# horovod/horovod

Hardware: AMD Instinct MI355X
Metric: images/sec, ResNet-50 synthetic (total over all GPUs) (higher is better)
Workload: dtype bf16; 1 GPU; model=resnet50, global_batch=64, image_size=224, parallelism=dp1, compression=none, reduction=average, optimizer=sgd, fused_sgd=True, fused_bn=False, hipgraph=False

## Files before the change

### csrc/bindings.cc

```cpp
#include <torch/extension.h>

#include "core.h"
#include "timeline.h"
#include "gpu.h"

namespace {

using namespace hvd;

ReduceOp OpFromInt(int op) { return (ReduceOp)op; }

py::tuple WaitHandle(int handle) {
  std::vector<at::Tensor> outputs;
  at::Tensor extra;
  int32_t result_int = -1;
  Status s;
  {
    py::gil_scoped_release nogil;
    s = State().handles.Wait(handle, outputs, extra, &result_int);
  }
  if (!s.ok()) {
    if (s.type == StatusType::ABORTED)
      throw std::runtime_error("HorovodInternalError: " + s.reason);
    throw std::runtime_error(s.reason);
// ... 201 lines not shown
          return hvd::gpu::FusedLarsStep(params, grads, momenta, lr, momentum,
                                         weight_decay, trust_coefficient, eps,
                                         nesterov, trust_clip, adapt,
                                         opt_tensor(grad_coef),
                                         opt_list(model_params),
                                         opt_tensor(skip));
        },
        py::arg("params"), py::arg("grads"), py::arg("momenta"),
        py::arg("lr"), py::arg("momentum"), py::arg("weight_decay"),
        py::arg("trust_coefficient"), py::arg("eps"), py::arg("nesterov"),
        py::arg("trust_clip"), py::arg("adapt"),
        py::arg("grad_coef") = py::none(),
        py::arg("model_params") = py::none(), py::arg("skip") = py::none());

  m.def("fused_bn_relu_forward",
        [](at::Tensor x, py::object residual, at::Tensor gamma, at::Tensor beta,
           at::Tensor rm, at::Tensor rv, double momentum, double eps) {
          at::Tensor res;
          if (!residual.is_none()) res = residual.cast<at::Tensor>();
          return hvd::gpu::FusedBnReluForward(x, res, gamma, beta, rm, rv,
                                              momentum, eps);
        });
  m.def("fused_bn_relu_backward",
        [](at::Tensor x, at::Tensor y, at::Tensor dy, at::Tensor mean,
           at::Tensor invstd, at::Tensor gamma, bool need_res) {
          return hvd::gpu::FusedBnReluBackward(x, y, dy, mean, invstd, gamma,
                                               need_res);
        });
  m.def("fused_bn_pass",
        [](int which, at::Tensor x, py::object a, py::object b, py::object out,
           at::Tensor mean, at::Tensor invstd, at::Tensor gamma,
           at::Tensor beta) {
          auto opt = [](const py::object& o) {
            return o.is_none() ? at::Tensor() : o.cast<at::Tensor>();
          };
          hvd::gpu::FusedBnPass(which, x, opt(a), opt(b), opt(out), mean,
                                invstd, gamma, beta);
        });

  m.def("sync_bn_stats",
        [](at::Tensor x) { return hvd::gpu::SyncBnStats(x); });
  m.def("sync_bn_normalize",
        [](at::Tensor x, at::Tensor stats, py::object weight, py::object bias,
           py::object rm, py::object rv, double momentum, double eps) {
          auto opt = [](const py::object& o) {
            return o.is_none() ? at::Tensor() : o.cast<at::Tensor>();
          };
          return hvd::gpu::SyncBnNormalize(x, stats, opt(weight), opt(bias),
                                           opt(rm), opt(rv), momentum, eps);
        });
  m.def("sync_bn_backward_reduce",
// ... 41 lines not shown
```

### csrc/bn_common.h

```cpp
#pragma once

#include <hip/hip_runtime.h>
#include <hip/hip_fp16.h>
#include <hip/hip_bf16.h>

#include <algorithm>
#include <cstdint>

#include "kernels.h"

namespace hvd {
namespace gpu {
namespace {

template <typename T>
__device__ __forceinline__ float to_f(T v) { return (float)v; }
template <>
__device__ __forceinline__ float to_f<__hip_bfloat16>(__hip_bfloat16 v) {
  return __bfloat162float(v);
}
template <typename T>
__device__ __forceinline__ T from_f(float v) { return (T)v; }
template <>
__device__ __forceinline__ __hip_bfloat16 from_f<__hip_bfloat16>(float v) {
  return __float2bfloat16(v);
}

template <typename T>
union Vec8 {
  uint4 u[2];
  T e[8];
  __device__ Vec8() {}
};

template <typename T>
__device__ __forceinline__ void load8(Vec8<T>& v, const T* p, long long i) {
  if (sizeof(T) == 2) {
    v.u[0] = ((const uint4*)p)[i];
  } else {
    v.u[0] = ((const uint4*)p)[i * 2];
    v.u[1] = ((const uint4*)p)[i * 2 + 1];
  }
}

template <typename T>
__device__ __forceinline__ void store8(T* p, long long i, const Vec8<T>& v) {
  if (sizeof(T) == 2) {
    ((uint4*)p)[i] = v.u[0];
// ... 80 lines not shown
```

### csrc/bn_kernels.hip

```cpp
#include "bn_common.h"
#include "kernels.h"

namespace hvd {
namespace gpu {

namespace {

template <typename T>
__global__ __launch_bounds__(256) void bn_stats_k(const T* __restrict__ x,
                                                  long long total, int C,
                                                  float* __restrict__ banks) {
  extern __shared__ float lds[];
  for (int c = threadIdx.x; c < 2 * C; c += blockDim.x) lds[c] = 0.f;
  __syncthreads();
  const long long tid = (long long)blockIdx.x * blockDim.x + threadIdx.x;
  const long long nthreads = (long long)gridDim.x * blockDim.x;
  const long long nvec = total / 8;
  const int c0 = octet_channel(C);
  float rsum[8] = {0}, rsq[8] = {0};
  auto add = [&](const Vec8<T>& v) {
#pragma unroll
    for (int k = 0; k < 8; ++k) {
      float f = to_f<T>(v.e[k]);
      rsum[k] += f;
// ... 21 lines not shown
}

template <typename T, bool ADD>
__global__ __launch_bounds__(256) void bn_apply_relu_k(
    const T* __restrict__ x, const T* __restrict__ res, T* __restrict__ y,
    const float* __restrict__ mean, const float* __restrict__ invstd,
    const float* __restrict__ gamma, const float* __restrict__ beta,
    long long total, int C) {
  const long long tid = (long long)blockIdx.x * blockDim.x + threadIdx.x;
  const long long nthreads = (long long)gridDim.x * blockDim.x;
  const long long nvec = total / 8;
  const int c0 = octet_channel(C);
  float rm[8], ri[8], rg[8], rb[8];
  load_octet(rm, mean, c0, 0.f);
  load_octet(ri, invstd, c0, 0.f);
  load_octet(rg, gamma, c0, 1.f);
  load_octet(rb, beta, c0, 0.f);
  for (long long i = tid; i < nvec; i += nthreads) {
    Vec8<T> vx, vr, vy;
    load8(vx, x, i);
    if (ADD) load8(vr, res, i);
#pragma unroll
    for (int k = 0; k < 8; ++k) {
      float f = (to_f<T>(vx.e[k]) - rm[k]) * ri[k] * rg[k] + rb[k];
      if (ADD) f += to_f<T>(vr.e[k]);
      vy.e[k] = from_f<T>(f > 0.f ? f : 0.f);
    }
    store8(y, i, vy);
  }
}

template <typename T, bool WRITE_G>
__global__ __launch_bounds__(256) void bn_bwd_stats_k(
    const T* __restrict__ x, const T* __restrict__ y, const T* __restrict__ dy,
    T* __restrict__ g_out, const float* __restrict__ mean,
    const float* __restrict__ invstd, long long total, int C,
    float* __restrict__ banks) {
  extern __shared__ float lds[];
  for (int c = threadIdx.x; c < 2 * C; c += blockDim.x) lds[c] = 0.f;
  __syncthreads();
  const long long tid = (long long)blockIdx.x * blockDim.x + threadIdx.x;
  const long long nthreads = (long long)gridDim.x * blockDim.x;
  const long long nvec = total / 8;
  const int c0 = octet_channel(C);
  float rmean[8], racc_g[8] = {0}, racc_gx[8] = {0};
  load_octet(rmean, mean, c0, 0.f);
  for (long long i = tid; i < nvec; i += nthreads) {
    Vec8<T> vx, vy, vd, vg;
    load8(vx, x, i);
    load8(vy, y, i);
    load8(vd, dy, i);
#pragma unroll
    for (int k = 0; k < 8; ++k) {
      float gv = to_f<T>(vy.e[k]) > 0.f ? to_f<T>(vd.e[k]) : 0.f;
      racc_g[k] += gv;
      racc_gx[k] += gv * (to_f<T>(vx.e[k]) - rmean[k]);
      if (WRITE_G) vg.e[k] = from_f<T>(gv);
    }
    if (WRITE_G) store8(g_out, i, vg);
  }
  float rinv[8];
  load_octet(rinv, invstd, c0, 0.f);
#pragma unroll
  for (int k = 0; k < 8; ++k) racc_gx[k] *= rinv[k];
  octet_flush(racc_g, racc_gx, c0, C, lds, banks);
}

__global__ __launch_bounds__(256) void bn_bank_reduce_k(float* banks,
                                                        int C) {
  for (int c = blockIdx.x * blockDim.x + threadIdx.x; c < 2 * C;
       c += gridDim.x * blockDim.x) {
    float acc = 0.f;
    for (int b = 0; b < kBnBanks; ++b) acc += banks[(size_t)b * 2 * C + c];
    banks[c] = acc;
  }
}

template <typename T, bool FROM_G>
__global__ __launch_bounds__(256) void bn_bwd_apply_k(
    const T* __restrict__ x, const T* __restrict__ y, const T* __restrict__ dy,
    T* __restrict__ dx, const float* __restrict__ mean,
    const float* __restrict__ invstd, const float* __restrict__ gamma,
    const float* __restrict__ sum_g, const float* __restrict__ sum_gx,
    long long total, int C, float inv_count) {
  const long long tid = (long long)blockIdx.x * blockDim.x + threadIdx.x;
  const long long nthreads = (long long)gridDim.x * blockDim.x;
  const long long nvec = total / 8;
  const int c0 = octet_channel(C);
  float rmean[8], rinv[8], rgi[8], rsg[8], rsgx[8];
  load_octet(rmean, mean, c0, 0.f);
  load_octet(rinv, invstd, c0, 0.f);
  load_octet(rgi, gamma, c0, 1.f);
  load_octet(rsg, sum_g, c0, 0.f);
  load_octet(rsgx, sum_gx, c0, 0.f);
#pragma unroll
  for (int k = 0; k < 8; ++k) {
    rgi[k] = rgi[k] * rinv[k];
    rsg[k] = rsg[k] * inv_count;
    rsgx[k] = rsgx[k] * inv_count;
  }
  for (long long i = tid; i < nvec; i += nthreads) {
    Vec8<T> vx, vy, vd, vo;
    load8(vx, x, i);
    if (!FROM_G) load8(vy, y, i);
    load8(vd, dy, i);
#pragma unroll
    for (int k = 0; k < 8; ++k) {
      float gv = FROM_G ? to_f<T>(vd.e[k])
                        : (to_f<T>(vy.e[k]) > 0.f ? to_f<T>(vd.e[k]) : 0.f);
      float xh = (to_f<T>(vx.e[k]) - rmean[k]) * rinv[k];
      float v = rgi[k] * (gv - rsg[k] - xh * rsgx[k]);
      vo.e[k] = from_f<T>(v);
    }
    store8(dx, i, vo);
  }
}

__global__ __launch_bounds__(256) void bn_finalize_k(
    const float* __restrict__ banks, float* __restrict__ mean,
    float* __restrict__ invstd, float* __restrict__ running_mean,
    float* __restrict__ running_var, long long count, float momentum,
    float eps, int C) {
  const int c = blockIdx.x * blockDim.x + threadIdx.x;
  if (c >= C) return;
  const float inv_n = 1.0f / (float)count;
  const float ub = count > 1 ? (float)count / (float)(count - 1) : 1.0f;
  float s = 0.f, q = 0.f;
#pragma unroll 16
  for (int b = 0; b < kBnBanks; ++b) {
    s += banks[(size_t)b * 2 * C + c];
    q += banks[(size_t)b * 2 * C + C + c];
  }
  float m = s * inv_n;
  float v = q * inv_n - m * m;
  mean[c] = m;
  invstd[c] = rsqrtf(v + eps);
  if (running_mean) {
    running_mean[c] = (1.f - momentum) * running_mean[c] + momentum * m;
    running_var[c] = (1.f - momentum) * running_var[c] + momentum * v * ub;
  }
}

template <size_t N>
bool aligned16(const void* const (&ptrs)[N]) {
  return aligned_to(ptrs, (int)N, 16);
}

}

#define DISPATCH_T(DT, FN)                                        \
  switch (DT) {                                                   \
    case DT_F32: { using scalar_t = float; FN; break; }           \
    case DT_F16: { using scalar_t = __half; FN; break; }          \
    case DT_BF16: { using scalar_t = __hip_bfloat16; FN; break; } \
    default: return hipErrorInvalidValue;                         \
  }

hipError_t BnFinalizeLaunch(const float* banks, float* mean, float* invstd,
                            float* running_mean, float* running_var,
                            long long count, float momentum, float eps,
                            int C, hipStream_t stream) {
  bn_finalize_k<<<(C + 255) / 256, 256, 0, stream>>>(
      banks, mean, invstd, running_mean, running_var, count, momentum, eps, C);
  return hipGetLastError();
}

hipError_t BnBankReduceLaunch(float* banks, int C, hipStream_t stream) {
  int blocks = (2 * C + 255) / 256;
  bn_bank_reduce_k<<<blocks, 256, 0, stream>>>(banks, C);
  return hipGetLastError();
}

hipError_t BnStatsLaunch(const void* x, long long total, int C, int dt,
                         float* banks, hipStream_t stream) {
  const void* const ptrs[] = {x};
  if (!aligned16(ptrs)) return hipErrorInvalidValue;
  int blocks = vec8_reduce_grid(total, C);
  size_t lds = 2 * (size_t)C * sizeof(float);
  DISPATCH_T(dt, (bn_stats_k<scalar_t><<<blocks, 256, lds, stream>>>(
                     (const scalar_t*)x, total, C, banks)));
  return hipGetLastError();
}

hipError_t BnApplyReluLaunch(const void* x, const void* res, void* y,
                             const float* mean, const float* invstd,
                             const float* gamma, const float* beta,
                             long long total, int C, int dt,
                             hipStream_t stream) {
  const void* const ptrs[] = {x, res, y, mean, invstd, gamma, beta};
  if (!aligned16(ptrs)) return hipErrorInvalidValue;
  int blocks = grid_for(total, C);
  if (res) {
    DISPATCH_T(dt, (bn_apply_relu_k<scalar_t, true><<<blocks, 256, 0, stream>>>(
                       (const scalar_t*)x, (const scalar_t*)res, (scalar_t*)y,
                       mean, invstd, gamma, beta, total, C)));
  } else {
    DISPATCH_T(dt,
               (bn_apply_relu_k<scalar_t, false><<<blocks, 256, 0, stream>>>(
                   (const scalar_t*)x, nullptr, (scalar_t*)y, mean, invstd,
                   gamma, beta, total, C)));
  }
  return hipGetLastError();
}

hipError_t BnBwdStatsLaunch(const void* x, const void* y, const void* dy,
                            void* g_out, const float* mean,
                            const float* invstd, long long total, int C,
                            int dt, float* banks, hipStream_t stream) {
  const void* const ptrs[] = {x, y, dy, g_out, mean, invstd};
  if (!aligned16(ptrs)) return hipErrorInvalidValue;
  int blocks = vec8_reduce_grid(total, C);
  size_t lds = 2 * (size_t)C * sizeof(float);
  if (g_out) {
    DISPATCH_T(dt,
               (bn_bwd_stats_k<scalar_t, true><<<blocks, 256, lds, stream>>>(
                   (const scalar_t*)x, (const scalar_t*)y, (const scalar_t*)dy,
                   (scalar_t*)g_out, mean, invstd, total, C, banks)));
  } else {
    DISPATCH_T(dt,
               (bn_bwd_stats_k<scalar_t, false><<<blocks, 256, lds, stream>>>(
                   (const scalar_t*)x, (const scalar_t*)y, (const scalar_t*)dy,
                   nullptr, mean, invstd, total, C, banks)));
  }
  return hipGetLastError();
}

hipError_t BnBwdApplyLaunch(const void* x, const void* y, const void* dy,
                            void* dx, const float* mean, const float* invstd,
                            const float* gamma, const float* sum_g,
                            const float* sum_gx, long long total, int C,
                            int dt, float inv_count, hipStream_t stream) {
  const void* const ptrs[] = {x,      y,     dy,    dx,    mean,
                              invstd, gamma, sum_g, sum_gx};
  if (!aligned16(ptrs)) return hipErrorInvalidValue;
  int blocks = grid_for(total, C);
  if (y) {
    DISPATCH_T(dt, (bn_bwd_apply_k<scalar_t, false><<<blocks, 256, 0, stream>>>(
                       (const scalar_t*)x, (const scalar_t*)y,
                       (const scalar_t*)dy, (scalar_t*)dx, mean, invstd, gamma,
                       sum_g, sum_gx, total, C, inv_count)));
  } else {
    DISPATCH_T(dt, (bn_bwd_apply_k<scalar_t, true><<<blocks, 256, 0, stream>>>(
                       (const scalar_t*)x, nullptr, (const scalar_t*)dy,
                       (scalar_t*)dx, mean, invstd, gamma, sum_g, sum_gx,
                       total, C, inv_count)));
  }
  return hipGetLastError();
}

#undef DISPATCH_T

}
}
```

### csrc/gpu.cc

```cpp
#include "gpu.h"

#include <hip/hip_runtime_api.h>
#include <rccl/rccl.h>
#include <roctracer/roctx.h>

#include <c10/hip/HIPCachingAllocator.h>
#include <c10/hip/HIPGuard.h>
#include <c10/hip/HIPStream.h>

#include <algorithm>
#include <condition_variable>
#include <cstring>
#include <deque>
#include <mutex>
#include <stdexcept>
#include <thread>
#include <unordered_map>

#include "core.h"
#include "hip_check.h"
#include "kernels.h"
#include "logging.h"
#include "timeline.h"

// ... 1323 lines not shown
    HIP_CHECK(AdasumDotsLaunch(args, dt, dots + start * 3, stream));
  }
  for (size_t start = 0; start < a.size(); start += kCopyBatchCapacity) {
    AdasumBatchArgs args;
    args.count = (int)std::min<size_t>(kCopyBatchCapacity, a.size() - start);
    for (int k = 0; k < args.count; ++k) {
      args.a[k] = a[start + k].data_ptr();
      args.b[k] = b[start + k].data_ptr();
      args.numel[k] = (unsigned long long)a[start + k].numel();
    }
    HIP_CHECK(AdasumScaledAddLaunch(args, dt, dots + start * 3, stream));
  }
}

namespace {

at::Tensor BnParamF32(const at::Tensor& t) {
  if (t.scalar_type() == at::kFloat && t.is_contiguous() &&
      (uintptr_t)t.data_ptr() % 16 == 0)
    return t;
  return t.to(at::kFloat).clone(at::MemoryFormat::Contiguous);
}

}

std::vector<at::Tensor> FusedBnReluForward(at::Tensor x, at::Tensor residual,
                                           at::Tensor gamma, at::Tensor beta,
                                           at::Tensor running_mean,
                                           at::Tensor running_var,
                                           double momentum, double eps) {
  TORCH_CHECK(x.dim() == 4, "fused BN expects NCHW logical 4-D input");
  TORCH_CHECK(x.is_contiguous(at::MemoryFormat::ChannelsLast),
              "fused BN requires channels_last layout");
  int64_t C = x.size(1);
  TORCH_CHECK(C % 8 == 0 && C <= 4096, "fused BN requires C % 8 == 0, C <= 4096");
  TORCH_CHECK(gamma.numel() == C && beta.numel() == C,
              "fused BN: weight and bias must have C elements");
  TORCH_CHECK(!residual.defined() ||
                  (residual.sizes() == x.sizes() &&
                   residual.scalar_type() == x.scalar_type() &&
                   residual.is_contiguous(at::MemoryFormat::ChannelsLast)),
              "fused BN: residual must match x in shape, dtype and layout");
  int device = (int)x.get_device();
  c10::hip::HIPGuard guard(device);
  hipStream_t stream = c10::hip::getCurrentHIPStream(device).stream();
  int64_t total = x.numel();
  int64_t count = total / C;
  int dt = (int)DataTypeFromTorch(x.scalar_type());

  auto fopts = at::TensorOptions().dtype(at::kFloat).device(x.device());
  const int64_t bank_elems = (int64_t)kBnBanks * 2 * C;
  at::Tensor ws = at::empty({bank_elems + 2 * C}, fopts);
  float* wsp = ws.data_ptr<float>();
  float* mean_p = wsp + bank_elems;
  float* invstd_p = mean_p + C;
  HIP_CHECK(hipMemsetAsync(wsp, 0, (size_t)bank_elems * sizeof(float),
                           stream));
  HIP_CHECK(BnStatsLaunch(x.data_ptr(), total, (int)C, dt, wsp, stream));
  TORCH_CHECK(!running_mean.defined() ||
                  (running_var.defined() && running_mean.numel() == C &&
                   running_var.numel() == C),
              "fused BN: running stats must have C elements");
  bool stats_f32 = running_mean.defined() &&
                   running_mean.scalar_type() == at::kFloat &&
                   running_mean.is_contiguous() &&
                   running_var.scalar_type() == at::kFloat &&
                   running_var.is_contiguous();
  HIP_CHECK(BnFinalizeLaunch(
      wsp, mean_p, invstd_p,
      stats_f32 ? running_mean.data_ptr<float>() : nullptr,
      stats_f32 ? running_var.data_ptr<float>() : nullptr, count,
      (float)momentum, (float)eps, (int)C, stream));
  at::Tensor mean = ws.narrow(0, bank_elems, C);
  at::Tensor invstd = ws.narrow(0, bank_elems + C, C);
  if (!stats_f32 && running_mean.defined()) {
    at::Tensor var = at::pow(invstd, -2) - eps;
    running_mean.mul_(1 - momentum).add_(mean.to(running_mean.scalar_type()),
                                         momentum);
    double ub = count > 1 ? (double)count / (count - 1) : 1.0;
    running_var.mul_(1 - momentum)
        .add_((var * ub).to(running_var.scalar_type()), momentum);
  }
  at::Tensor gamma_f = BnParamF32(gamma);
  at::Tensor beta_f = BnParamF32(beta);
  at::Tensor y = at::empty_like(x);
  HIP_CHECK(BnApplyReluLaunch(
      x.data_ptr(), residual.defined() ? residual.data_ptr() : nullptr,
      y.data_ptr(), mean_p, invstd_p, gamma_f.data_ptr<float>(),
      beta_f.data_ptr<float>(), total, (int)C, dt, stream));
  return {y, mean, invstd};
}

std::vector<at::Tensor> FusedBnReluBackward(at::Tensor x, at::Tensor y,
                                            at::Tensor dy, at::Tensor mean,
                                            at::Tensor invstd, at::Tensor gamma,
                                            bool need_residual_grad) {
  int device = (int)x.get_device();
  c10::hip::HIPGuard guard(device);
  hipStream_t stream = c10::hip::getCurrentHIPStream(device).stream();
  int64_t C = x.size(1);
  int64_t total = x.numel();
  int64_t count = total / C;
  int dt = (int)DataTypeFromTorch(x.scalar_type());
  if (!dy.is_contiguous(at::MemoryFormat::ChannelsLast))
    dy = dy.contiguous(at::MemoryFormat::ChannelsLast);
  TORCH_CHECK(x.dim() == 4 && C % 8 == 0 && C <= 4096 &&
                  x.is_contiguous(at::MemoryFormat::ChannelsLast) &&
                  y.is_contiguous(at::MemoryFormat::ChannelsLast),
              "fused BN backward: x and y must be channels_last with "
              "C % 8 == 0, C <= 4096");
  TORCH_CHECK(y.sizes() == x.sizes() && dy.sizes() == x.sizes() &&
                  y.scalar_type() == x.scalar_type() &&
                  dy.scalar_type() == x.scalar_type() &&
                  mean.numel() == C && invstd.numel() == C &&
                  gamma.numel() == C,
              "fused BN backward: mismatched shapes or dtypes");

  auto fopts = at::TensorOptions().dtype(at::kFloat).device(x.device());
  at::Tensor sums = at::empty({(int64_t)kBnBanks * 2 * C}, fopts);
  float* bankp = sums.data_ptr<float>();
  HIP_CHECK(hipMemsetAsync(bankp, 0,
                           (size_t)kBnBanks * 2 * C * sizeof(float), stream));
  at::Tensor dres;
  if (need_residual_grad) dres = at::empty_like(x);
  at::Tensor mean_f = BnParamF32(mean), invstd_f = BnParamF32(invstd);
  HIP_CHECK(BnBwdStatsLaunch(x.data_ptr(), y.data_ptr(), dy.data_ptr(),
                             need_residual_grad ? dres.data_ptr() : nullptr,
                             mean_f.data_ptr<float>(),
                             invstd_f.data_ptr<float>(), total, (int)C, dt,
                             bankp, stream));
  HIP_CHECK(BnBankReduceLaunch(bankp, (int)C, stream));
  at::Tensor gamma_f = BnParamF32(gamma);
  at::Tensor dx = at::empty_like(x);
  HIP_CHECK(BnBwdApplyLaunch(
      x.data_ptr(), need_residual_grad ? nullptr : y.data_ptr(),
      need_residual_grad ? dres.data_ptr() : dy.data_ptr(), dx.data_ptr(),
      mean_f.data_ptr<float>(), invstd_f.data_ptr<float>(),
      gamma_f.data_ptr<float>(), bankp, bankp + C, total, (int)C, dt,
      (float)(1.0 / count), stream));
  at::Tensor sum_g = sums.narrow(0, 0, C), sum_gx = sums.narrow(0, C, C);
  at::Tensor dbeta = gamma.scalar_type() == at::kFloat
                         ? sum_g
                         : sum_g.to(gamma.scalar_type());
  at::Tensor dgamma = gamma.scalar_type() == at::kFloat
                          ? sum_gx
                          : sum_gx.to(gamma.scalar_type());
  std::vector<at::Tensor> out{dx, dgamma, dbeta};
  if (need_residual_grad) out.push_back(dres);
  return out;
}

void FusedBnPass(int which, at::Tensor x, at::Tensor a, at::Tensor b,
                 at::Tensor out, at::Tensor mean, at::Tensor invstd,
                 at::Tensor gamma, at::Tensor beta) {
  TORCH_CHECK(x.dim() == 4 && x.is_contiguous(at::MemoryFormat::ChannelsLast),
              "fused BN requires channels_last layout");
  int64_t C = x.size(1);
  TORCH_CHECK(C % 8 == 0 && C <= 4096, "fused BN requires C % 8 == 0, C <= 4096");
  for (const at::Tensor* t : {&a, &b, &out})
    TORCH_CHECK(!t->defined() ||
                    (t->sizes() == x.sizes() &&
                     t->scalar_type() == x.scalar_type() &&
// ... 14 lines not shown
  const size_t bank_bytes = (size_t)kBnBanks * 2 * C * sizeof(float);
  at::Tensor banks = at::empty(
      {(int64_t)kBnBanks * 2 * C},
      at::TensorOptions().dtype(at::kFloat).device(x.device()));
  float* bankp = banks.data_ptr<float>();
  const float* mp = mean.data_ptr<float>();
  const float* ip = invstd.data_ptr<float>();
  switch (which) {
    case 0:
      HIP_CHECK(hipMemsetAsync(bankp, 0, bank_bytes, stream));
      HIP_CHECK(BnStatsLaunch(x.data_ptr(), total, (int)C, dt, bankp, stream));
      break;
    case 1:
      TORCH_CHECK(out.defined(), "fused BN pass 1 needs out");
      HIP_CHECK(BnApplyReluLaunch(x.data_ptr(), ptr(a), out.data_ptr(), mp, ip,
                                  gamma.data_ptr<float>(),
                                  beta.data_ptr<float>(), total, (int)C, dt,
                                  stream));
      break;
    case 2:
      TORCH_CHECK(a.defined() && b.defined(), "fused BN pass 2 needs y, dy");
      HIP_CHECK(hipMemsetAsync(bankp, 0, bank_bytes, stream));
      HIP_CHECK(BnBwdStatsLaunch(x.data_ptr(), a.data_ptr(), b.data_ptr(),
                                 ptr(out), mp, ip, total, (int)C, dt, bankp,
                                 stream));
      break;
    case 3:
      TORCH_CHECK(b.defined() && out.defined(),
                  "fused BN pass 3 needs dy and out");
      HIP_CHECK(BnBwdApplyLaunch(x.data_ptr(), ptr(a), b.data_ptr(),
                                 out.data_ptr(), mp, ip,
                                 gamma.data_ptr<float>(), mp, ip, total,
                                 (int)C, dt, 1.0f / (float)(total / C),
                                 stream));
      break;
    default:
      TORCH_CHECK(false, "fused BN pass: which must be 0..3");
  }
}

namespace {

struct SbnShape {
  int64_t outer, C, inner;
  bool channels_last;
  at::MemoryFormat format;
};

SbnShape SyncBnShape(const at::Tensor& x) {
  TORCH_CHECK(x.is_cuda(), "sync_bn: expected a GPU tensor");
  TORCH_CHECK(x.dim() >= 2 && x.numel() > 0,
              "sync_bn: expected a non-empty input of at least 2 dims");
  auto st = x.scalar_type();
  TORCH_CHECK(st == at::kFloat || st == at::kHalf || st == at::kBFloat16,
              "sync_bn: input must be fp32, fp16 or bf16");
  SbnShape s;
  s.C = x.size(1);
  s.format = at::MemoryFormat::Contiguous;
  s.channels_last = false;
  if (!x.is_contiguous()) {
// ... 227 lines not shown
```

### csrc/gpu.h

```cpp
#pragma once

#include <cstdint>
#include <optional>
#include <vector>

#include <ATen/ATen.h>

namespace hvd {
struct GlobalState;
struct Response;
struct TensorTableEntry;

namespace gpu {

uintptr_t RecordReadyEvent(int device);

void Execute(GlobalState& st, Response& resp,
             std::vector<TensorTableEntry>& entries);

void WaitAllPending();
void Shutdown();

void AbortComms(const std::string& why);
bool CommsFailed();

void SetOneshotThreshold(int64_t bytes);

bool RcclUsed();

void AdasumCombine(std::vector<at::Tensor>& a, std::vector<at::Tensor>& b);

std::vector<at::Tensor> FusedBnReluForward(at::Tensor x, at::Tensor residual,
                                           at::Tensor gamma, at::Tensor beta,
                                           at::Tensor running_mean,
                                           at::Tensor running_var,
                                           double momentum, double eps);
std::vector<at::Tensor> FusedBnReluBackward(at::Tensor x, at::Tensor y,
                                            at::Tensor dy, at::Tensor mean,
                                            at::Tensor invstd, at::Tensor gamma,
                                            bool need_residual_grad);
void FusedBnPass(int which, at::Tensor x, at::Tensor a, at::Tensor b,
                 at::Tensor out, at::Tensor mean, at::Tensor invstd,
                 at::Tensor gamma, at::Tensor beta);

at::Tensor SyncBnStats(at::Tensor x);
std::vector<at::Tensor> SyncBnNormalize(at::Tensor x, at::Tensor stats,
                                        at::Tensor weight, at::Tensor bias,
                                        at::Tensor running_mean,
                                        at::Tensor running_var,
                                        double momentum, double eps);
at::Tensor SyncBnBackwardReduce(at::Tensor x, at::Tensor dy, at::Tensor mean,
                                at::Tensor invstd);
at::Tensor SyncBnBackwardApply(at::Tensor x, at::Tensor dy, at::Tensor mean,
                               at::Tensor invstd, at::Tensor weight,
                               at::Tensor sums, at::Tensor count);

at::Tensor MultiTensorGradNorm(std::vector<at::Tensor>& grads,
                               double max_norm);
at::Tensor MultiTensorScaledGradNorm(
    std::vector<at::Tensor>& grads, std::optional<double> max_norm,
    at::Tensor scale = at::Tensor(), at::Tensor found_inf = at::Tensor(),
    at::Tensor growth_tracker = at::Tensor(), double growth_factor = 1.0,
    double backoff_factor = 1.0, int64_t growth_interval = 0);
// ... 44 lines not shown
```

### csrc/kernels.h

```cpp
#pragma once

#include <hip/hip_runtime.h>

#include <type_traits>

namespace hvd {
namespace gpu {

enum KDType {
  DT_U8 = 0,
  DT_I8 = 1,
  DT_I32 = 2,
  DT_I64 = 3,
  DT_F16 = 4,
  DT_F32 = 5,
  DT_F64 = 6,
  DT_BOOL = 7,
  DT_BF16 = 8,
  DT_U16 = 9,
  DT_I16 = 10,
};

constexpr int kCopyBatchCapacity = 48;

// ... 174 lines not shown

hipError_t LarsNormsLaunch(const LarsBatchArgs& args, const float* grad_coef,
                           const float* skip, float* partials,
                           hipStream_t stream);
hipError_t LarsTrustLaunch(const LarsBatchArgs& args, const LarsScalars& s,
                           const float* partials, const float* skip,
                           float* trust, hipStream_t stream);
hipError_t LarsUpdateLaunch(const LarsBatchArgs& args, const LarsScalars& s,
                            const float* grad_coef, const float* trust,
                            const float* skip, hipStream_t stream);
hipError_t LarsNormsMasterLaunch(const LarsMasterBatchArgs& args, int dt,
                                 const float* grad_coef, const float* skip,
                                 float* partials, hipStream_t stream);
hipError_t LarsTrustLaunch(const LarsMasterBatchArgs& args,
                           const LarsScalars& s, const float* partials,
                           const float* skip, float* trust,
                           hipStream_t stream);
hipError_t LarsUpdateMasterLaunch(const LarsMasterBatchArgs& args, int dt,
                                  const LarsScalars& s,
                                  const float* grad_coef, const float* trust,
                                  const float* skip, hipStream_t stream);

constexpr int kBnBanks = 64;

hipError_t BnStatsLaunch(const void* x, long long total, int C, int dt,
                         float* banks, hipStream_t stream);
hipError_t BnFinalizeLaunch(const float* banks, float* mean, float* invstd,
                            float* running_mean, float* running_var,
                            long long count, float momentum, float eps,
                            int C, hipStream_t stream);
hipError_t BnBankReduceLaunch(float* banks, int C, hipStream_t stream);
hipError_t BnApplyReluLaunch(const void* x, const void* res, void* y,
                             const float* mean, const float* invstd,
                             const float* gamma, const float* beta,
                             long long total, int C, int dt,
                             hipStream_t stream);
hipError_t BnBwdStatsLaunch(const void* x, const void* y, const void* dy,
                            void* g_out, const float* mean,
                            const float* invstd, long long total, int C,
                            int dt, float* banks, hipStream_t stream);
hipError_t BnBwdApplyLaunch(const void* x, const void* y, const void* dy,
                            void* dx, const float* mean, const float* invstd,
                            const float* gamma, const float* sum_g,
                            const float* sum_gx, long long total, int C,
                            int dt, float inv_count, hipStream_t stream);

bool SyncBnBanked(long long C, long long inner);
hipError_t SyncBnStatsLaunch(const void* x, long long outer, long long C,
                             long long inner, int dt, float* banks, float* out,
                             hipStream_t stream);
hipError_t SyncBnFinalizeLaunch(const float* stats, float* mean, float* invstd,
                                float* running_mean, float* running_var,
                                float momentum, float eps, int C,
                                hipStream_t stream);
hipError_t SyncBnApplyLaunch(const void* x, void* y, const float* mean,
                             const float* invstd, const float* w,
                             const float* b, long long outer, long long C,
                             long long inner, int dt, hipStream_t stream);
hipError_t SyncBnBwdReduceLaunch(const void* x, const void* dy,
                                 const float* mean, const float* invstd,
                                 long long outer, long long C, long long inner,
                                 int dt, float* banks, float* out,
                                 hipStream_t stream);
hipError_t SyncBnBwdApplyLaunch(const void* x, const void* dy, void* dx,
                                const float* mean, const float* invstd,
                                const float* w, const float* sums,
                                const float* count, long long outer,
                                long long C, long long inner, int dt,
// ... 5 lines not shown
```

### horovod_amd/ops/fused_bn.py

```python
import torch
import torch.nn.functional as F

from horovod_amd import _core


def _fusable(x):
    return (x.is_cuda and x.dim() == 4 and
            x.is_contiguous(memory_format=torch.channels_last) and
            x.size(1) % 8 == 0 and x.size(1) <= 4096 and
            x.dtype in (torch.float32, torch.float16, torch.bfloat16))


class _FusedBNReLUFn(torch.autograd.Function):
    @staticmethod
    def forward(ctx, x, residual, weight, bias, running_mean, running_var,
                momentum, eps):
        y, mean, invstd = _core.fused_bn_relu_forward(
            x, residual, weight, bias, running_mean, running_var, momentum,
            eps)
        ctx.save_for_backward(x, y, mean, invstd, weight)
        ctx.has_residual = residual is not None
        return y

    @staticmethod
    def backward(ctx, dy):
        x, y, mean, invstd, weight = ctx.saved_tensors
        outs = _core.fused_bn_relu_backward(x, y, dy, mean, invstd, weight,
                                            ctx.has_residual)
        dx, dgamma, dbeta = outs[0], outs[1], outs[2]
        dres = outs[3] if ctx.has_residual else None
        return dx, dres, dgamma, dbeta, None, None, None, None


class FusedBNReLU(torch.nn.BatchNorm2d):

    def forward(self, input):
        if self.training and _fusable(input):
            return _FusedBNReLUFn.apply(
                input.contiguous(memory_format=torch.channels_last), None,
                self.weight, self.bias, self.running_mean, self.running_var,
                self.momentum if self.momentum is not None else 0.1, self.eps)
        return F.relu(super().forward(input))


class FusedBNAddReLU(torch.nn.BatchNorm2d):

    def forward(self, input, residual):
        if self.training and _fusable(input) and _fusable(residual) and \
                residual.shape == input.shape and residual.dtype == input.dtype:
            return _FusedBNReLUFn.apply(
                input.contiguous(memory_format=torch.channels_last),
# ... 5 lines not shown
```

Measured before the change: 5658 images/sec.

## Recompute ReLU mask from input in fused BN backward and reuse persistent banks

For non-residual BN+ReLU, backward now rebuilds the ReLU mask from x, mean, invstd, gamma and beta instead of saving and rereading the output y. This cuts one activation read per backward kernel and frees the saved y earlier. Reduction banks are kept in a persistent per-stream buffer and zeroed by the reduce/finalize kernels, replacing a per-call allocation and memset. The cost is extra arithmetic and a per-stream lock, with a fallback path used under graph capture.

```diff
diff --git a/csrc/bindings.cc b/csrc/bindings.cc
--- a/csrc/bindings.cc
+++ b/csrc/bindings.cc
@@ -247,11 +247,19 @@
                                               momentum, eps);
         });
   m.def("fused_bn_relu_backward",
-        [](at::Tensor x, at::Tensor y, at::Tensor dy, at::Tensor mean,
-           at::Tensor invstd, at::Tensor gamma, bool need_res) {
-          return hvd::gpu::FusedBnReluBackward(x, y, dy, mean, invstd, gamma,
-                                               need_res);
-        });
+        [](at::Tensor x, py::object y, at::Tensor dy, at::Tensor mean,
+           at::Tensor invstd, at::Tensor gamma, bool need_res,
+           py::object beta) {
+          auto opt = [](const py::object& o) {
+            return o.is_none() ? at::Tensor() : o.cast<at::Tensor>();
+          };
+          return hvd::gpu::FusedBnReluBackward(x, opt(y), dy, mean, invstd,
+                                               gamma, need_res, opt(beta));
+        },
+        py::arg("x"), py::arg("y"), py::arg("dy"), py::arg("mean"),
+        py::arg("invstd"), py::arg("gamma"), py::arg("need_residual_grad"),
+        py::arg("beta") = py::none());
+  m.def("fused_bn_lean_path", []() { return hvd::gpu::FusedBnLeanPath(); });
   m.def("fused_bn_pass",
         [](int which, at::Tensor x, py::object a, py::object b, py::object out,
            at::Tensor mean, at::Tensor invstd, at::Tensor gamma,
diff --git a/csrc/bn_common.h b/csrc/bn_common.h
--- a/csrc/bn_common.h
+++ b/csrc/bn_common.h
@@ -24,6 +24,16 @@
 template <>
 __device__ __forceinline__ __hip_bfloat16 from_f<__hip_bfloat16>(float v) {
   return __float2bfloat16(v);
+}
+
+__device__ __forceinline__ float bn_preact(float x, float mean, float invstd,
+                                           float gamma, float beta) {
+  return fmaf(__fmul_rn(__fsub_rn(x, mean), invstd), gamma, beta);
+}
+
+template <typename T>
+__device__ __forceinline__ bool bn_relu_mask(float f) {
+  return to_f<T>(from_f<T>(f)) > 0.f;
 }
 
 template <typename T>
diff --git a/csrc/bn_kernels.hip b/csrc/bn_kernels.hip
--- a/csrc/bn_kernels.hip
+++ b/csrc/bn_kernels.hip
@@ -67,7 +67,7 @@
     if (ADD) load8(vr, res, i);
 #pragma unroll
     for (int k = 0; k < 8; ++k) {
-      float f = (to_f<T>(vx.e[k]) - rm[k]) * ri[k] * rg[k] + rb[k];
+      float f = bn_preact(to_f<T>(vx.e[k]), rm[k], ri[k], rg[k], rb[k]);
       if (ADD) f += to_f<T>(vr.e[k]);
       vy.e[k] = from_f<T>(f > 0.f ? f : 0.f);
     }
@@ -75,11 +75,12 @@
   }
 }
 
-template <typename T, bool WRITE_G>
+template <typename T, bool WRITE_G, bool FROM_X>
 __global__ __launch_bounds__(256) void bn_bwd_stats_k(
     const T* __restrict__ x, const T* __restrict__ y, const T* __restrict__ dy,
     T* __restrict__ g_out, const float* __restrict__ mean,
-    const float* __restrict__ invstd, long long total, int C,
+    const float* __restrict__ invstd, const float* __restrict__ gamma,
+    const float* __restrict__ beta, long long total, int C,
     float* __restrict__ banks) {
   extern __shared__ float lds[];
   for (int c = threadIdx.x; c < 2 * C; c += blockDim.x) lds[c] = 0.f;
@@ -90,79 +91,105 @@
   const int c0 = octet_channel(C);
   float rmean[8], racc_g[8] = {0}, racc_gx[8] = {0};
   load_octet(rmean, mean, c0, 0.f);
+  float rinv[8], rg[8], rb[8];
+  if (FROM_X) {
+    load_octet(rinv, invstd, c0, 0.f);
+    load_octet(rg, gamma, c0, 1.f);
+    load_octet(rb, beta, c0, 0.f);
+  }
   for (long long i = tid; i < nvec; i += nthreads) {
     Vec8<T> vx, vy, vd, vg;
     load8(vx, x, i);
-    load8(vy, y, i);
+    if (!FROM_X) load8(vy, y, i);
     load8(vd, dy, i);
 #pragma unroll
     for (int k = 0; k < 8; ++k) {
-      float gv = to_f<T>(vy.e[k]) > 0.f ? to_f<T>(vd.e[k]) : 0.f;
+      const float xf = to_f<T>(vx.e[k]);
+      const bool on =
+          FROM_X ? bn_relu_mask<T>(bn_preact(xf, rmean[k], rinv[k], rg[k], rb[k]))
+                 : to_f<T>(vy.e[k]) > 0.f;
+      float gv = on ? to_f<T>(vd.e[k]) : 0.f;
       racc_g[k] += gv;
-      racc_gx[k] += gv * (to_f<T>(vx.e[k]) - rmean[k]);
+      racc_gx[k] += gv * (xf - rmean[k]);
       if (WRITE_G) vg.e[k] = from_f<T>(gv);
     }
     if (WRITE_G) store8(g_out, i, vg);
   }
-  float rinv[8];
-  load_octet(rinv, invstd, c0, 0.f);
+  if (!FROM_X) load_octet(rinv, invstd, c0, 0.f);
 #pragma unroll
   for (int k = 0; k < 8; ++k) racc_gx[k] *= rinv[k];
   octet_flush(racc_g, racc_gx, c0, C, lds, banks);
 }
 
+template <bool CLEAR>
 __global__ __launch_bounds__(256) void bn_bank_reduce_k(float* banks,
-                                                        int C) {
+                                                        float* sums, int C) {
   for (int c = blockIdx.x * blockDim.x + threadIdx.x; c < 2 * C;
        c += gridDim.x * blockDim.x) {
     float acc = 0.f;
     for (int b = 0; b < kBnBanks; ++b) acc += banks[(size_t)b * 2 * C + c];
-    banks[c] = acc;
-  }
-}
-
-template <typename T, bool FROM_G>
+    if (CLEAR)
+      for (int b = 0; b < kBnBanks; ++b) banks[(size_t)b * 2 * C + c] = 0.f;
+    sums[c] = acc;
+  }
+}
+
+template <typename T, bool FROM_G, bool FROM_X>
 __global__ __launch_bounds__(256) void bn_bwd_apply_k(
     const T* __restrict__ x, const T* __restrict__ y, const T* __restrict__ dy,
     T* __restrict__ dx, const float* __restrict__ mean,
     const float* __restrict__ invstd, const float* __restrict__ gamma,
-    const float* __restrict__ sum_g, const float* __restrict__ sum_gx,
-    long long total, int C, float inv_count) {
+    const float* __restrict__ beta, const float* __restrict__ sum_g,
+    const float* __restrict__ sum_gx, long long total, int C,
+    float inv_count) {
+  static_assert(!(FROM_G && FROM_X), "one source of the ReLU mask");
   const long long tid = (long long)blockIdx.x * blockDim.x + threadIdx.x;
   const long long nthreads = (long long)gridDim.x * blockDim.x;
   const long long nvec = total / 8;
   const int c0 = octet_channel(C);
-  float rmean[8], rinv[8], rgi[8], rsg[8], rsgx[8];
+  float rmean[8], rinv[8], rgi[8], rsg[8], rsgx[8], rb[8];
   load_octet(rmean, mean, c0, 0.f);
   load_octet(rinv, invstd, c0, 0.f);
   load_octet(rgi, gamma, c0, 1.f);
   load_octet(rsg, sum_g, c0, 0.f);
   load_octet(rsgx, sum_gx, c0, 0.f);
+  if (FROM_X) load_octet(rb, beta, c0, 0.f);
 #pragma unroll
   for (int k = 0; k < 8; ++k) {
-    rgi[k] = rgi[k] * rinv[k];
+    if (!FROM_X) rgi[k] = rgi[k] * rinv[k];
     rsg[k] = rsg[k] * inv_count;
     rsgx[k] = rsgx[k] * inv_count;
   }
   for (long long i = tid; i < nvec; i += nthreads) {
     Vec8<T> vx, vy, vd, vo;
     load8(vx, x, i);
-    if (!FROM_G) load8(vy, y, i);
+    if (!FROM_G && !FROM_X) load8(vy, y, i);
     load8(vd, dy, i);
 #pragma unroll
     for (int k = 0; k < 8; ++k) {
-      float gv = FROM_G ? to_f<T>(vd.e[k])
-                        : (to_f<T>(vy.e[k]) > 0.f ? to_f<T>(vd.e[k]) : 0.f);
-      float xh = (to_f<T>(vx.e[k]) - rmean[k]) * rinv[k];
-      float v = rgi[k] * (gv - rsg[k] - xh * rsgx[k]);
+      const float xf = to_f<T>(vx.e[k]);
+      float gv;
+      if (FROM_G) {
+        gv = to_f<T>(vd.e[k]);
+      } else {
+        const bool on =
+            FROM_X ? bn_relu_mask<T>(
+                         bn_preact(xf, rmean[k], rinv[k], rgi[k], rb[k]))
+                   : to_f<T>(vy.e[k]) > 0.f;
+        gv = on ? to_f<T>(vd.e[k]) : 0.f;
+      }
+      float xh = (xf - rmean[k]) * rinv[k];
+      const float gi = FROM_X ? rgi[k] * rinv[k] : rgi[k];
+      float v = gi * (gv - rsg[k] - xh * rsgx[k]);
       vo.e[k] = from_f<T>(v);
     }
     store8(dx, i, vo);
   }
 }
 
+template <bool CLEAR>
 __global__ __launch_bounds__(256) void bn_finalize_k(
-    const float* __restrict__ banks, float* __restrict__ mean,
+    float* __restrict__ banks, float* __restrict__ mean,
     float* __restrict__ invstd, float* __restrict__ running_mean,
     float* __restrict__ running_var, long long count, float momentum,
     float eps, int C) {
@@ -176,6 +203,13 @@
     s += banks[(size_t)b * 2 * C + c];
     q += banks[(size_t)b * 2 * C + C + c];
   }
+  if (CLEAR) {
+#pragma unroll 16
+    for (int b = 0; b < kBnBanks; ++b) {
+      banks[(size_t)b * 2 * C + c] = 0.f;
+      banks[(size_t)b * 2 * C + C + c] = 0.f;
+    }
+  }
   float m = s * inv_n;
   float v = q * inv_n - m * m;
   mean[c] = m;
@@ -201,18 +235,31 @@
     default: return hipErrorInvalidValue;                         \
   }
 
-hipError_t BnFinalizeLaunch(const float* banks, float* mean, float* invstd,
+hipError_t BnFinalizeLaunch(float* banks, float* mean, float* invstd,
                             float* running_mean, float* running_var,
                             long long count, float momentum, float eps,
-                            int C, hipStream_t stream) {
-  bn_finalize_k<<<(C + 255) / 256, 256, 0, stream>>>(
-      banks, mean, invstd, running_mean, running_var, count, momentum, eps, C);
-  return hipGetLastError();
-}
-
-hipError_t BnBankReduceLaunch(float* banks, int C, hipStream_t stream) {
+                            int C, bool clear_banks, hipStream_t stream) {
+  const int blocks = (C + 255) / 256;
+  if (clear_banks)
+    bn_finalize_k<true><<<blocks, 256, 0, stream>>>(
+        banks, mean, invstd, running_mean, running_var, count, momentum, eps,
+        C);
+  else
+    bn_finalize_k<false><<<blocks, 256, 0, stream>>>(
+        banks, mean, invstd, running_mean, running_var, count, momentum, eps,
+        C);
+  return hipGetLastError();
+}
+
+hipError_t BnBankReduceLaunch(float* banks, float* sums, int C,
+                              bool clear_banks, hipStream_t stream) {
+  const void* const ptrs[] = {sums};
+  if (!aligned16(ptrs)) return hipErrorInvalidValue;
   int blocks = (2 * C + 255) / 256;
-  bn_bank_reduce_k<<<blocks, 256, 0, stream>>>(banks, C);
+  if (clear_banks)
+    bn_bank_reduce_k<true><<<blocks, 256, 0, stream>>>(banks, sums, C);
+  else
+    bn_bank_reduce_k<false><<<blocks, 256, 0, stream>>>(banks, sums, C);
   return hipGetLastError();
 }
 
@@ -250,45 +297,63 @@
 
 hipError_t BnBwdStatsLaunch(const void* x, const void* y, const void* dy,
                             void* g_out, const float* mean,
-                            const float* invstd, long long total, int C,
-                            int dt, float* banks, hipStream_t stream) {
-  const void* const ptrs[] = {x, y, dy, g_out, mean, invstd};
-  if (!aligned16(ptrs)) return hipErrorInvalidValue;
+                            const float* invstd, const float* gamma,
+                            const float* beta, long long total, int C, int dt,
+                            float* banks, hipStream_t stream) {
+  const void* const ptrs[] = {x, y, dy, g_out, mean, invstd, gamma, beta};
+  if (!aligned16(ptrs)) return hipErrorInvalidValue;
+  if (beta ? (g_out != nullptr || !gamma) : !y) return hipErrorInvalidValue;
   int blocks = vec8_reduce_grid(total, C);
   size_t lds = 2 * (size_t)C * sizeof(float);
-  if (g_out) {
-    DISPATCH_T(dt,
-               (bn_bwd_stats_k<scalar_t, true><<<blocks, 256, lds, stream>>>(
-                   (const scalar_t*)x, (const scalar_t*)y, (const scalar_t*)dy,
-                   (scalar_t*)g_out, mean, invstd, total, C, banks)));
+  if (beta) {
+    DISPATCH_T(
+        dt, (bn_bwd_stats_k<scalar_t, false, true><<<blocks, 256, lds, stream>>>(
+                (const scalar_t*)x, nullptr, (const scalar_t*)dy, nullptr, mean,
+                invstd, gamma, beta, total, C, banks)));
+  } else if (g_out) {
+    DISPATCH_T(
+        dt, (bn_bwd_stats_k<scalar_t, true, false><<<blocks, 256, lds, stream>>>(
+                (const scalar_t*)x, (const scalar_t*)y, (const scalar_t*)dy,
+                (scalar_t*)g_out, mean, invstd, nullptr, nullptr, total, C,
+                banks)));
   } else {
-    DISPATCH_T(dt,
-               (bn_bwd_stats_k<scalar_t, false><<<blocks, 256, lds, stream>>>(
-                   (const scalar_t*)x, (const scalar_t*)y, (const scalar_t*)dy,
-                   nullptr, mean, invstd, total, C, banks)));
+    DISPATCH_T(
+        dt,
+        (bn_bwd_stats_k<scalar_t, false, false><<<blocks, 256, lds, stream>>>(
+            (const scalar_t*)x, (const scalar_t*)y, (const scalar_t*)dy,
+            nullptr, mean, invstd, nullptr, nullptr, total, C, banks)));
   }
   return hipGetLastError();
 }
 
 hipError_t BnBwdApplyLaunch(const void* x, const void* y, const void* dy,
                             void* dx, const float* mean, const float* invstd,
-                            const float* gamma, const float* sum_g,
-                            const float* sum_gx, long long total, int C,
-                            int dt, float inv_count, hipStream_t stream) {
-  const void* const ptrs[] = {x,      y,     dy,    dx,    mean,
-                              invstd, gamma, sum_g, sum_gx};
+                            const float* gamma, const float* beta,
+                            const float* sum_g, const float* sum_gx,
+                            long long total, int C, int dt, float inv_count,
+                            hipStream_t stream) {
+  const void* const ptrs[] = {x,     y,    dy,    dx,    mean, invstd,
+                              gamma, beta, sum_g, sum_gx};
   if (!aligned16(ptrs)) return hipErrorInvalidValue;
   int blocks = grid_for(total, C);
-  if (y) {
-    DISPATCH_T(dt, (bn_bwd_apply_k<scalar_t, false><<<blocks, 256, 0, stream>>>(
-                       (const scalar_t*)x, (const scalar_t*)y,
-                       (const scalar_t*)dy, (scalar_t*)dx, mean, invstd, gamma,
-                       sum_g, sum_gx, total, C, inv_count)));
+  if (beta) {
+    DISPATCH_T(
+        dt, (bn_bwd_apply_k<scalar_t, false, true><<<blocks, 256, 0, stream>>>(
+                (const scalar_t*)x, nullptr, (const scalar_t*)dy,
+                (scalar_t*)dx, mean, invstd, gamma, beta, sum_g, sum_gx, total,
+                C, inv_count)));
+  } else if (y) {
+    DISPATCH_T(
+        dt, (bn_bwd_apply_k<scalar_t, false, false><<<blocks, 256, 0, stream>>>(
+                (const scalar_t*)x, (const scalar_t*)y, (const scalar_t*)dy,
+                (scalar_t*)dx, mean, invstd, gamma, nullptr, sum_g, sum_gx,
+                total, C, inv_count)));
   } else {
-    DISPATCH_T(dt, (bn_bwd_apply_k<scalar_t, true><<<blocks, 256, 0, stream>>>(
-                       (const scalar_t*)x, nullptr, (const scalar_t*)dy,
-                       (scalar_t*)dx, mean, invstd, gamma, sum_g, sum_gx,
-                       total, C, inv_count)));
+    DISPATCH_T(
+        dt, (bn_bwd_apply_k<scalar_t, true, false><<<blocks, 256, 0, stream>>>(
+                (const scalar_t*)x, nullptr, (const scalar_t*)dy,
+                (scalar_t*)dx, mean, invstd, gamma, nullptr, sum_g, sum_gx,
+                total, C, inv_count)));
   }
   return hipGetLastError();
 }
diff --git a/csrc/gpu.cc b/csrc/gpu.cc
--- a/csrc/gpu.cc
+++ b/csrc/gpu.cc
@@ -1369,7 +1369,74 @@
   return t.to(at::kFloat).clone(at::MemoryFormat::Contiguous);
 }
 
-}
+bool BnLeanPath() {
+  static const bool on = [] {
+    const char* v = std::getenv("HOROVOD_FUSED_BN_WORKSPACE");
+    return !(v && v[0] == '0' && v[1] == '\0');
+  }();
+  return on;
+}
+
+struct BnBankSlot {
+  std::mutex mu;
+  at::Tensor banks;
+};
+
+BnBankSlot* BnSlot(int device, hipStream_t stream) {
+  static std::mutex mu;
+  static auto* slots = new std::unordered_map<uint64_t, std::unordered_map<
+                           hipStream_t, BnBankSlot*>>();
+  std::lock_guard<std::mutex> lock(mu);
+  BnBankSlot*& slot = (*slots)[(uint64_t)device][stream];
+  if (!slot) slot = new BnBankSlot();
+  return slot;
+}
+
+class BnBankLease {
+ public:
+  BnBankLease(int device, hipStream_t stream, int64_t C,
+              const at::TensorOptions& fopts) {
+    hipStreamCaptureStatus st = hipStreamCaptureStatusNone;
+    if (BnLeanPath()) HIP_CHECK(hipStreamIsCapturing(stream, &st));
+    if (BnLeanPath() && st == hipStreamCaptureStatusNone) {
+      slot_ = BnSlot(device, stream);
+      lock_ = std::unique_lock<std::mutex>(slot_->mu);
+      if (!slot_->banks.defined())
+        slot_->banks =
+            at::zeros({(int64_t)kBnBanks * 2 * kBnMaxChannels}, fopts);
+      banks_ = slot_->banks.data_ptr<float>();
+    } else {
+      own_ = at::empty({(int64_t)kBnBanks * 2 * C}, fopts);
+      banks_ = own_.data_ptr<float>();
+      HIP_CHECK(hipMemsetAsync(banks_, 0,
+                               (size_t)kBnBanks * 2 * C * sizeof(float),
+                               stream));
+    }
+  }
+  ~BnBankLease() {
+    if (slot_ && !consumed_) slot_->banks = at::Tensor();
+  }
+  BnBankLease(const BnBankLease&) = delete;
+  BnBankLease& operator=(const BnBankLease&) = delete;
+
+  float* banks() const { return banks_; }
+  bool persistent() const { return slot_ != nullptr; }
+  void Consumed() {
+    consumed_ = true;
+    if (lock_.owns_lock()) lock_.unlock();
+  }
+
+ private:
+  BnBankSlot* slot_ = nullptr;
+  std::unique_lock<std::mutex> lock_;
+  at::Tensor own_;
+  float* banks_ = nullptr;
+  bool consumed_ = false;
+};
+
+}
+
+bool FusedBnLeanPath() { return BnLeanPath(); }
 
 std::vector<at::Tensor> FusedBnReluForward(at::Tensor x, at::Tensor residual,
                                            at::Tensor gamma, at::Tensor beta,
@@ -1396,14 +1463,6 @@
   int dt = (int)DataTypeFromTorch(x.scalar_type());
 
   auto fopts = at::TensorOptions().dtype(at::kFloat).device(x.device());
-  const int64_t bank_elems = (int64_t)kBnBanks * 2 * C;
-  at::Tensor ws = at::empty({bank_elems + 2 * C}, fopts);
-  float* wsp = ws.data_ptr<float>();
-  float* mean_p = wsp + bank_elems;
-  float* invstd_p = mean_p + C;
-  HIP_CHECK(hipMemsetAsync(wsp, 0, (size_t)bank_elems * sizeof(float),
-                           stream));
-  HIP_CHECK(BnStatsLaunch(x.data_ptr(), total, (int)C, dt, wsp, stream));
   TORCH_CHECK(!running_mean.defined() ||
                   (running_var.defined() && running_mean.numel() == C &&
                    running_var.numel() == C),
@@ -1413,13 +1472,20 @@
                    running_mean.is_contiguous() &&
                    running_var.scalar_type() == at::kFloat &&
                    running_var.is_contiguous();
+  at::Tensor stats = at::empty({2 * C}, fopts);
+  float* mean_p = stats.data_ptr<float>();
+  float* invstd_p = mean_p + C;
+  BnBankLease lease(device, stream, C, fopts);
+  HIP_CHECK(
+      BnStatsLaunch(x.data_ptr(), total, (int)C, dt, lease.banks(), stream));
   HIP_CHECK(BnFinalizeLaunch(
-      wsp, mean_p, invstd_p,
+      lease.banks(), mean_p, invstd_p,
       stats_f32 ? running_mean.data_ptr<float>() : nullptr,
       stats_f32 ? running_var.data_ptr<float>() : nullptr, count,
-      (float)momentum, (float)eps, (int)C, stream));
-  at::Tensor mean = ws.narrow(0, bank_elems, C);
-  at::Tensor invstd = ws.narrow(0, bank_elems + C, C);
+      (float)momentum, (float)eps, (int)C, lease.persistent(), stream));
+  lease.Consumed();
+  at::Tensor mean = stats.narrow(0, 0, C);
+  at::Tensor invstd = stats.narrow(0, C, C);
   if (!stats_f32 && running_mean.defined()) {
     at::Tensor var = at::pow(invstd, -2) - eps;
     running_mean.mul_(1 - momentum).add_(mean.to(running_mean.scalar_type()),
@@ -1441,7 +1507,8 @@
 std::vector<at::Tensor> FusedBnReluBackward(at::Tensor x, at::Tensor y,
                                             at::Tensor dy, at::Tensor mean,
                                             at::Tensor invstd, at::Tensor gamma,
-                                            bool need_residual_grad) {
+                                            bool need_residual_grad,
+                                            at::Tensor beta) {
   int device = (int)x.get_device();
   c10::hip::HIPGuard guard(device);
   hipStream_t stream = c10::hip::getCurrentHIPStream(device).stream();
@@ -1449,42 +1516,54 @@
   int64_t total = x.numel();
   int64_t count = total / C;
   int dt = (int)DataTypeFromTorch(x.scalar_type());
+  const bool from_x = beta.defined() && !need_residual_grad && BnLeanPath();
   if (!dy.is_contiguous(at::MemoryFormat::ChannelsLast))
     dy = dy.contiguous(at::MemoryFormat::ChannelsLast);
+  TORCH_CHECK(from_x || y.defined(),
+              "fused BN backward: y is needed unless beta is given, no "
+              "residual gradient is wanted and HOROVOD_FUSED_BN_WORKSPACE "
+              "is not 0");
   TORCH_CHECK(x.dim() == 4 && C % 8 == 0 && C <= 4096 &&
                   x.is_contiguous(at::MemoryFormat::ChannelsLast) &&
-                  y.is_contiguous(at::MemoryFormat::ChannelsLast),
+                  (from_x || y.is_contiguous(at::MemoryFormat::ChannelsLast)),
               "fused BN backward: x and y must be channels_last with "
               "C % 8 == 0, C <= 4096");
-  TORCH_CHECK(y.sizes() == x.sizes() && dy.sizes() == x.sizes() &&
-                  y.scalar_type() == x.scalar_type() &&
+  TORCH_CHECK((from_x || (y.sizes() == x.sizes() &&
+                          y.scalar_type() == x.scalar_type())) &&
+                  dy.sizes() == x.sizes() &&
                   dy.scalar_type() == x.scalar_type() &&
                   mean.numel() == C && invstd.numel() == C &&
-                  gamma.numel() == C,
+                  gamma.numel() == C && (!from_x || beta.numel() == C),
               "fused BN backward: mismatched shapes or dtypes");
 
   auto fopts = at::TensorOptions().dtype(at::kFloat).device(x.device());
-  at::Tensor sums = at::empty({(int64_t)kBnBanks * 2 * C}, fopts);
-  float* bankp = sums.data_ptr<float>();
-  HIP_CHECK(hipMemsetAsync(bankp, 0,
-                           (size_t)kBnBanks * 2 * C * sizeof(float), stream));
+  at::Tensor sums = at::empty({2 * C}, fopts);
+  float* sump = sums.data_ptr<float>();
   at::Tensor dres;
   if (need_residual_grad) dres = at::empty_like(x);
   at::Tensor mean_f = BnParamF32(mean), invstd_f = BnParamF32(invstd);
-  HIP_CHECK(BnBwdStatsLaunch(x.data_ptr(), y.data_ptr(), dy.data_ptr(),
-                             need_residual_grad ? dres.data_ptr() : nullptr,
-                             mean_f.data_ptr<float>(),
-                             invstd_f.data_ptr<float>(), total, (int)C, dt,
-                             bankp, stream));
-  HIP_CHECK(BnBankReduceLaunch(bankp, (int)C, stream));
-  at::Tensor gamma_f = BnParamF32(gamma);
+  at::Tensor gamma_f = BnParamF32(gamma), beta_f;
+  if (from_x) beta_f = BnParamF32(beta);
+  const float* gamma_p = gamma_f.data_ptr<float>();
+  const float* beta_p = from_x ? beta_f.data_ptr<float>() : nullptr;
   at::Tensor dx = at::empty_like(x);
+  {
+    BnBankLease lease(device, stream, C, fopts);
+    HIP_CHECK(BnBwdStatsLaunch(
+        x.data_ptr(), from_x ? nullptr : y.data_ptr(), dy.data_ptr(),
+        need_residual_grad ? dres.data_ptr() : nullptr,
+        mean_f.data_ptr<float>(), invstd_f.data_ptr<float>(),
+        from_x ? gamma_p : nullptr, beta_p, total, (int)C, dt, lease.banks(),
+        stream));
+    HIP_CHECK(BnBankReduceLaunch(lease.banks(), sump, (int)C,
+                                 lease.persistent(), stream));
+    lease.Consumed();
+  }
   HIP_CHECK(BnBwdApplyLaunch(
-      x.data_ptr(), need_residual_grad ? nullptr : y.data_ptr(),
+      x.data_ptr(), (need_residual_grad || from_x) ? nullptr : y.data_ptr(),
       need_residual_grad ? dres.data_ptr() : dy.data_ptr(), dx.data_ptr(),
-      mean_f.data_ptr<float>(), invstd_f.data_ptr<float>(),
-      gamma_f.data_ptr<float>(), bankp, bankp + C, total, (int)C, dt,
-      (float)(1.0 / count), stream));
+      mean_f.data_ptr<float>(), invstd_f.data_ptr<float>(), gamma_p, beta_p,
+      sump, sump + C, total, (int)C, dt, (float)(1.0 / count), stream));
   at::Tensor sum_g = sums.narrow(0, 0, C), sum_gx = sums.narrow(0, C, C);
   at::Tensor dbeta = gamma.scalar_type() == at::kFloat
                          ? sum_g
@@ -1545,20 +1624,38 @@
       TORCH_CHECK(a.defined() && b.defined(), "fused BN pass 2 needs y, dy");
       HIP_CHECK(hipMemsetAsync(bankp, 0, bank_bytes, stream));
       HIP_CHECK(BnBwdStatsLaunch(x.data_ptr(), a.data_ptr(), b.data_ptr(),
-                                 ptr(out), mp, ip, total, (int)C, dt, bankp,
-                                 stream));
+                                 ptr(out), mp, ip, nullptr, nullptr, total,
+                                 (int)C, dt, bankp, stream));
       break;
     case 3:
       TORCH_CHECK(b.defined() && out.defined(),
                   "fused BN pass 3 needs dy and out");
       HIP_CHECK(BnBwdApplyLaunch(x.data_ptr(), ptr(a), b.data_ptr(),
                                  out.data_ptr(), mp, ip,
-                                 gamma.data_ptr<float>(), mp, ip, total,
+                                 gamma.data_ptr<float>(), nullptr, mp, ip,
+                                 total, (int)C, dt,
+                                 1.0f / (float)(total / C), stream));
+      break;
+    case 4:
+      TORCH_CHECK(b.defined(), "fused BN pass 4 needs dy");
+      HIP_CHECK(hipMemsetAsync(bankp, 0, bank_bytes, stream));
+      HIP_CHECK(BnBwdStatsLaunch(x.data_ptr(), nullptr, b.data_ptr(), nullptr,
+                                 mp, ip, gamma.data_ptr<float>(),
+                                 beta.data_ptr<float>(), total, (int)C, dt,
+                                 bankp, stream));
+      break;
+    case 5:
+      TORCH_CHECK(b.defined() && out.defined(),
+                  "fused BN pass 5 needs dy and out");
+      HIP_CHECK(BnBwdApplyLaunch(x.data_ptr(), nullptr, b.data_ptr(),
+                                 out.data_ptr(), mp, ip,
+                                 gamma.data_ptr<float>(),
+                                 beta.data_ptr<float>(), mp, ip, total,
                                  (int)C, dt, 1.0f / (float)(total / C),
                                  stream));
       break;
     default:
-      TORCH_CHECK(false, "fused BN pass: which must be 0..3");
+      TORCH_CHECK(false, "fused BN pass: which must be 0..5");
   }
 }
 
diff --git a/csrc/gpu.h b/csrc/gpu.h
--- a/csrc/gpu.h
+++ b/csrc/gpu.h
@@ -38,7 +38,9 @@
 std::vector<at::Tensor> FusedBnReluBackward(at::Tensor x, at::Tensor y,
                                             at::Tensor dy, at::Tensor mean,
                                             at::Tensor invstd, at::Tensor gamma,
-                                            bool need_residual_grad);
+                                            bool need_residual_grad,
+                                            at::Tensor beta = at::Tensor());
+bool FusedBnLeanPath();
 void FusedBnPass(int which, at::Tensor x, at::Tensor a, at::Tensor b,
                  at::Tensor out, at::Tensor mean, at::Tensor invstd,
                  at::Tensor gamma, at::Tensor beta);
diff --git a/csrc/kernels.h b/csrc/kernels.h
--- a/csrc/kernels.h
+++ b/csrc/kernels.h
@@ -220,14 +220,16 @@
                                   const float* skip, hipStream_t stream);
 
 constexpr int kBnBanks = 64;
+constexpr int kBnMaxChannels = 4096;
 
 hipError_t BnStatsLaunch(const void* x, long long total, int C, int dt,
                          float* banks, hipStream_t stream);
-hipError_t BnFinalizeLaunch(const float* banks, float* mean, float* invstd,
+hipError_t BnFinalizeLaunch(float* banks, float* mean, float* invstd,
                             float* running_mean, float* running_var,
                             long long count, float momentum, float eps,
-                            int C, hipStream_t stream);
-hipError_t BnBankReduceLaunch(float* banks, int C, hipStream_t stream);
+                            int C, bool clear_banks, hipStream_t stream);
+hipError_t BnBankReduceLaunch(float* banks, float* sums, int C,
+                              bool clear_banks, hipStream_t stream);
 hipError_t BnApplyReluLaunch(const void* x, const void* res, void* y,
                              const float* mean, const float* invstd,
                              const float* gamma, const float* beta,
@@ -235,13 +237,15 @@
                              hipStream_t stream);
 hipError_t BnBwdStatsLaunch(const void* x, const void* y, const void* dy,
                             void* g_out, const float* mean,
-                            const float* invstd, long long total, int C,
-                            int dt, float* banks, hipStream_t stream);
+                            const float* invstd, const float* gamma,
+                            const float* beta, long long total, int C, int dt,
+                            float* banks, hipStream_t stream);
 hipError_t BnBwdApplyLaunch(const void* x, const void* y, const void* dy,
                             void* dx, const float* mean, const float* invstd,
-                            const float* gamma, const float* sum_g,
-                            const float* sum_gx, long long total, int C,
-                            int dt, float inv_count, hipStream_t stream);
+                            const float* gamma, const float* beta,
+                            const float* sum_g, const float* sum_gx,
+                            long long total, int C, int dt, float inv_count,
+                            hipStream_t stream);
 
 bool SyncBnBanked(long long C, long long inner);
 hipError_t SyncBnStatsLaunch(const void* x, long long outer, long long C,
diff --git a/horovod_amd/ops/fused_bn.py b/horovod_amd/ops/fused_bn.py
--- a/horovod_amd/ops/fused_bn.py
+++ b/horovod_amd/ops/fused_bn.py
@@ -11,6 +11,9 @@
             x.dtype in (torch.float32, torch.float16, torch.bfloat16))
 
 
+_LEAN = _core.fused_bn_lean_path()
+
+
 class _FusedBNReLUFn(torch.autograd.Function):
     @staticmethod
     def forward(ctx, x, residual, weight, bias, running_mean, running_var,
@@ -18,15 +21,24 @@
         y, mean, invstd = _core.fused_bn_relu_forward(
             x, residual, weight, bias, running_mean, running_var, momentum,
             eps)
-        ctx.save_for_backward(x, y, mean, invstd, weight)
         ctx.has_residual = residual is not None
+        ctx.from_x = _LEAN and residual is None
+        if ctx.from_x:
+            ctx.save_for_backward(x, mean, invstd, weight, bias)
+        else:
+            ctx.save_for_backward(x, y, mean, invstd, weight)
         return y
 
     @staticmethod
     def backward(ctx, dy):
-        x, y, mean, invstd, weight = ctx.saved_tensors
-        outs = _core.fused_bn_relu_backward(x, y, dy, mean, invstd, weight,
-                                            ctx.has_residual)
+        if ctx.from_x:
+            x, mean, invstd, weight, bias = ctx.saved_tensors
+            outs = _core.fused_bn_relu_backward(x, None, dy, mean, invstd,
+                                                weight, False, bias)
+        else:
+            x, y, mean, invstd, weight = ctx.saved_tensors
+            outs = _core.fused_bn_relu_backward(x, y, dy, mean, invstd,
+                                                weight, ctx.has_residual)
         dx, dgamma, dbeta = outs[0], outs[1], outs[2]
         dres = outs[3] if ctx.has_residual else None
         return dx, dres, dgamma, dbeta, None, None, None, None
```

New measurement: 5750 images/sec, median of 6. 1.02x the previous value.
